# thu-ml/stochastic_gcn

Hardware: AMD Instinct MI355X
Metric: training edges/s (SpMM) (higher is better)
Workload: dtype f32

## Files before the change

### stochastic_gcn_amd/csrc/sgcn_gemm.hip

```cpp
#include "sgcn_dev.h"
#include "sgcn_bwd.h"

namespace sgcn {

typedef float f16acc __attribute__((ext_vector_type(16)));

constexpr int kTM = 32, kTN = 128, kTK = 32;

struct GemmArgs {
    const float* A; int64_t lda;
    const float* B; int64_t ldb;
    float* C; int64_t ldc;
    int32_t M, N, K;
    int32_t accumulate;
    int32_t kchunk;
    float* ws;
    const float* offset; const float* scale; float eps; int32_t relu;
    float* xhat; float* rstd;
    int32_t epi;
    const float* A2; int64_t lda2; int32_t a_split;
    DropArgs drop_a;
    DropArgs drop_c;
    int32_t vec_a, vec_b;
    const int32_t* a_gidx;
    const int32_t* a_gidx2;
};

__device__ __forceinline__ float wsum(float v) {
#pragma unroll
    for (int o = 32; o > 0; o >>= 1) v += __shfl_xor(v, o, 64);
    return v;
}

constexpr int kAsFloats = kTM * (kTK + 1), kBsFloats = kTK * (kTN + 4);
constexpr int kGroupFloats = kAsFloats + kBsFloats;

template <bool TA, bool TB, int KG>
__device__ __forceinline__ void gemm_body(const GemmArgs& g, const int bx, const int by, const int bz) {
    extern __shared__ float smem[];
    const int kg = threadIdx.x / kBlock;
    const int tid = threadIdx.x % kBlock, lane = tid & 63, wave = tid >> 6;
    float (*As)[kTK + 1] = reinterpret_cast<float (*)[kTK + 1]>(smem + kg * kGroupFloats);
    float (*Bs)[kTN + 4] = reinterpret_cast<float (*)[kTN + 4]>(smem + kg * kGroupFloats + kAsFloats);
    const int m0 = bx * kTM, n0 = by * kTN;
    const int kbeg = bz * g.kchunk;
    const int kend = min(g.K, kbeg + g.kchunk);
    f16acc acc = {};
    float ra[4], rb[16];
    float ep_scale[2] = {1.f, 1.f}, ep_offset[2] = {0.f, 0.f};
    if (g.epi == 2) {
#pragma unroll
        for (int e = 0; e < 2; e++) {
            const int c = (threadIdx.x & 63) + e * kWave;
            if (c < g.N) { ep_scale[e] = g.scale[c]; ep_offset[e] = g.offset[c]; }
        }
    }

    auto ld4 = [&](const float* rowp, bool vec, bool rowok, int first, int limit, float* out) {
        if (vec) {
            const bool ok = rowok && first + 3 < limit;
            const float4 v = *reinterpret_cast<const float4*>(rowp + (ok ? first : 0));
            out[0] = ok ? v.x : 0.f; out[1] = ok ? v.y : 0.f; out[2] = ok ? v.z : 0.f; out[3] = ok ? v.w : 0.f;
        } else {
#pragma unroll
            for (int e = 0; e < 4; e++) {
                const bool ok = rowok && first + e < limit;
                const float v = rowp[ok ? first + e : 0];
                out[e] = ok ? v : 0.f;
            }
        }
    };
    const float* arow = nullptr;
    if (!TA) {
        const int row = min(m0 + (tid >> 3), g.M - 1);
        if (g.A2 && row >= g.a_split) {
            const int r2 = row - g.a_split;
            arow = g.A2 + (int64_t)(g.a_gidx2 ? g.a_gidx2[r2] : r2) * g.lda2;
        } else {
            arow = g.A + (int64_t)(g.a_gidx ? g.a_gidx[row] : row) * g.lda;
        }
    }
    auto fetch = [&](int k0) {
        if (!TA) {
            const int i = tid >> 3, kq = (tid & 7) * 4, row = m0 + i;
            ld4(arow, g.vec_a, row < g.M, k0 + kq, kend, ra);
            if (g.drop_a.on) {
#pragma unroll
                for (int e = 0; e < 4; e++) ra[e] *= drop_factor(g.drop_a, row, k0 + kq + e);
            }
        } else {
            const int kk = tid >> 3, iq = (tid & 7) * 4, k = k0 + kk, kc = min(k, kend - 1);
            const int64_t ak = g.a_gidx ? g.a_gidx[kc] : kc;
            ld4(g.A + ak * g.lda, g.vec_a, k < kend, m0 + iq, g.M, ra);
            if (g.drop_a.on) {
#pragma unroll
                for (int e = 0; e < 4; e++) ra[e] *= drop_factor(g.drop_a, k, m0 + iq + e);
            }
        }
        if (!TB) {
#pragma unroll
            for (int r = 0; r < 4; r++) {
                const int kk = (tid >> 5) + 8 * r, jq = (tid & 31) * 4, k = k0 + kk;
                ld4(g.B + (int64_t)min(k, kend - 1) * g.ldb, g.vec_b, k < kend, n0 + jq, g.N, rb + r * 4);
            }
        } else {
#pragma unroll
            for (int r = 0; r < 4; r++) {
                const int j = (tid >> 3) + 32 * r, kq = (tid & 7) * 4, col = n0 + j;
                ld4(g.B + (int64_t)min(col, g.N - 1) * g.ldb, g.vec_b, col < g.N, k0 + kq, kend, rb + r * 4);
            }
        }
    };
    auto stage = [&]() {
        if (!TA) {
            const int i = tid >> 3, kq = (tid & 7) * 4;
#pragma unroll
            for (int e = 0; e < 4; e++) As[i][kq + e] = ra[e];
        } else {
            const int kk = tid >> 3, iq = (tid & 7) * 4;
#pragma unroll
            for (int e = 0; e < 4; e++) As[iq + e][kk] = ra[e];
        }
        if (!TB) {
#pragma unroll
            for (int r = 0; r < 4; r++) {
                const int kk = (tid >> 5) + 8 * r, jq = (tid & 31) * 4;
                *reinterpret_cast<float4*>(&Bs[kk][jq]) = make_float4(rb[r * 4], rb[r * 4 + 1], rb[r * 4 + 2], rb[r * 4 + 3]);
            }
        } else {
#pragma unroll
            for (int r = 0; r < 4; r++) {
                const int j = (tid >> 3) + 32 * r, kq = (tid & 7) * 4;
#pragma unroll
                for (int e = 0; e < 4; e++) Bs[kq + e][j] = rb[r * 4 + e];
            }
        }
    };

    const int iters = ((kend - kbeg + kTK - 1) / kTK + KG - 1) / KG;
    if (iters > 0) fetch(kbeg + kg * kTK);
    for (int it = 0; it < iters; it++) {
        const int k0 = kbeg + (it * KG + kg) * kTK;
        stage();
        __syncthreads();
        if (it + 1 < iters) fetch(k0 + KG * kTK);
        const int fi = lane & 31, fk = lane >> 5;
#pragma unroll
        for (int kk2 = 0; kk2 < kTK / 2; kk2++) {
            const float a = As[fi][kk2 * 2 + fk];
            const float b = Bs[kk2 * 2 + fk][wave * 32 + fi];
            acc = __builtin_amdgcn_mfma_f32_32x32x2f32(a, b, acc, 0, 0, 0);
        }
        __syncthreads();
    }

    const int cj = wave * 32 + (lane & 31);
    if (KG > 1) {
        if (kg > 0) {
#pragma unroll
            for (int r = 0; r < 16; r++) Bs[(r & 3) + 8 * (r >> 2) + 4 * (lane >> 5)][cj] = acc[r];
        }
        __syncthreads();
        if (kg == 0) {
            for (int o = 1; o < KG; o++) {
                float (*P)[kTN + 4] = reinterpret_cast<float (*)[kTN + 4]>(smem + o * kGroupFloats + kAsFloats);
#pragma unroll
                for (int r = 0; r < 16; r++) acc[r] += P[(r & 3) + 8 * (r >> 2) + 4 * (lane >> 5)][cj];
            }
        }
    }
    if (g.epi == 0) {
        if (kg != 0) return;
        float* base = g.ws ? g.ws + (int64_t)bz * g.M * g.N : g.C;
        const int64_t ld = g.ws ? g.N : g.ldc;
        const bool add = !g.ws && g.accumulate;
#pragma unroll
        for (int r = 0; r < 16; r++) {
            const int row = m0 + (r & 3) + 8 * (r >> 2) + 4 * (lane >> 5), col = n0 + cj;
            if (row < g.M && col < g.N) {
                float* p = base + (int64_t)row * ld + col;
                float v = acc[r];
                if (g.drop_c.on) v *= drop_factor(g.drop_c, row, col);
                *p = add ? *p + v : v;
            }
        }
        return;
    }
    float (*Cs)[kTN + 4] = reinterpret_cast<float (*)[kTN + 4]>(smem + kAsFloats);
    if (KG > 1) __syncthreads();
    if (kg == 0) {
#pragma unroll
        for (int r = 0; r < 16; r++) Cs[(r & 3) + 8 * (r >> 2) + 4 * (lane >> 5)][cj] = acc[r];
    }
    __syncthreads();
    for (int rr = kg * (kBlock / kWave) + wave; rr < kTM; rr += KG * (kBlock / kWave)) {
        const int row = m0 + rr;
        if (row >= g.M) break;
        float* yr = g.C + (int64_t)row * g.ldc;
        if (g.epi == 1) {
            for (int c = lane; c < g.N; c += kWave) { const float v = Cs[rr][c]; yr[c] = g.relu ? fmaxf(v, 0.f) : v; }
            continue;
        }
        float s = 0.f;
        for (int c = lane; c < g.N; c += kWave) s += Cs[rr][c];
        const float mean = wsum(s) / (float)g.N;
        float q = 0.f;
        for (int c = lane; c < g.N; c += kWave) { const float t = Cs[rr][c] - mean; q += t * t; }
        const float rs = rsqrtf(wsum(q) / (float)g.N + g.eps);
        if (lane == 0) g.rstd[row] = rs;
        float* hr = g.xhat + (int64_t)row * g.N;
#pragma unroll
        for (int e = 0; e < 2; e++) {
            const int c = lane + e * kWave;
            if (c < g.N) {
                const float h = (Cs[rr][c] - mean) * rs;
                hr[c] = h;
                const float v = h * ep_scale[e] + ep_offset[e];
                yr[c] = g.relu ? fmaxf(v, 0.f) : v;
            }
        }
    }
}

template <bool TA, bool TB, int KG>
__global__ __launch_bounds__(kBlock * KG) void gemm_kernel(GemmArgs g) {
    gemm_body<TA, TB, KG>(g, (int)blockIdx.x, (int)blockIdx.y, (int)blockIdx.z);
}

struct GemmGroup {
    GemmArgs g[kMaxGroup];
    int32_t first[kMaxGroup + 1];
    int32_t gx[kMaxGroup], gy[kMaxGroup];
    int32_t n;
};

template <bool TA, bool TB, int KG>
__global__ __launch_bounds__(kBlock * KG) void gemm_group_kernel(GemmGroup G) {
    const int b = (int)blockIdx.x;
    int j = 0;
#pragma unroll
    for (int q = 1; q < kMaxGroup; q++) j += (q < G.n && b >= G.first[q]) ? 1 : 0;
    const int l = b - G.first[j];
    const int gx = G.gx[j], gy = G.gy[j];
    gemm_body<TA, TB, KG>(G.g[j], l % gx, (l / gx) % gy, l / (gx * gy));
}

__global__ void splitk_reduce_kernel(const float* __restrict__ ws, int32_t S, int32_t M, int32_t N,
                                     float* __restrict__ C, int64_t ldc, int32_t accumulate) {
    const int64_t i = (int64_t)blockIdx.x * blockDim.x + threadIdx.x;
    const int64_t mn = (int64_t)M * N;
    if (i >= mn) return;
    float s = 0.f;
    for (int z = 0; z < S; z++) s += ws[(int64_t)z * mn + i];
    float* p = C + (i / N) * ldc + (i % N);
    *p = accumulate ? *p + s : s;
}

__global__ void dense_bwd_reduce_kernel(ReduceJob j, int32_t gemm_blocks, const float* __restrict__ ln_partial,
                                        int32_t nblk, int32_t d, float* __restrict__ doffset,
                                        float* __restrict__ dscale, int32_t ln_accumulate) {
    if ((int)blockIdx.x < gemm_blocks) {
        const int64_t i = (int64_t)blockIdx.x * blockDim.x + threadIdx.x;
        const int64_t mn = (int64_t)j.M * j.N;
        if (i >= mn) return;
        float s = 0.f;
        for (int z = 0; z < j.S; z++) s += j.ws[(int64_t)z * mn + i];
        float* p = j.C + (i / j.N) * j.ldc + (i % j.N);
        *p = j.accumulate ? *p + s : s;
    } else {
        ln_param_reduce_cols32(ln_partial, nblk, d, doffset, dscale, (int)blockIdx.x - gemm_blocks, ln_accumulate != 0);
    }
}

__global__ void dense_bwd_reduce_multi_kernel(ReduceMulti R) { reduce_multi_body(R, (int)blockIdx.x, nullptr); }

__global__ __launch_bounds__(kBlock) void splitk_ln_act_kernel(const float* __restrict__ ws, int32_t S,
                                                               GemmArgs g) {
    const int lane = threadIdx.x & 63;
    const int64_t row = (int64_t)blockIdx.x * (kBlock / kWave) + threadIdx.x / kWave;
    if (row >= g.M) return;
    const int64_t mn = (int64_t)g.M * g.N;
    float v[2];
    float sc[2] = {1.f, 1.f}, of[2] = {0.f, 0.f};
    if (g.epi == 2) {
#pragma unroll
        for (int e = 0; e < 2; e++) {
            const int c = lane + e * kWave;
            if (c < g.N) { sc[e] = g.scale[c]; of[e] = g.offset[c]; }
        }
    }
#pragma unroll
    for (int e = 0; e < 2; e++) {
        const int c = lane + e * kWave;
        float s = 0.f;
        if (c < g.N)
            for (int z = 0; z < S; z++) s += ws[(int64_t)z * mn + row * g.N + c];
        v[e] = s;
    }
    float* yr = g.C + row * g.ldc;
    if (g.epi == 2) {
        const float mean = wsum(v[0] + v[1]) / (float)g.N;
        float q = 0.f;
#pragma unroll
        for (int e = 0; e < 2; e++) if (lane + e * kWave < g.N) { const float t = v[e] - mean; q += t * t; }
        const float rs = rsqrtf(wsum(q) / (float)g.N + g.eps);
        if (lane == 0) g.rstd[row] = rs;
#pragma unroll
        for (int e = 0; e < 2; e++) {
            const int c = lane + e * kWave;
            if (c < g.N) {
                const float h = (v[e] - mean) * rs;
                g.xhat[row * g.N + c] = h;
                const float y = h * sc[e] + of[e];
                yr[c] = g.relu ? fmaxf(y, 0.f) : y;
            }
        }
    } else {
#pragma unroll
        for (int e = 0; e < 2; e++) {
            const int c = lane + e * kWave;
            if (c < g.N) yr[c] = (g.epi == 1 && g.relu) ? fmaxf(v[e], 0.f) : v[e];
        }
    }
}


struct RowDense {
    const float* W; int64_t ldw; int32_t N, kg;
    const float* offset; const float* scale; float eps; int32_t relu, epi;
    DropArgs drop;
    float* Y; int64_t ldy; float* xhat; float* rstd;
};

__global__ __launch_bounds__(kBlock) void splitk_ln_dense_kernel(const float* __restrict__ ws, int32_t S, GemmArgs g, RowDense d) {
    extern __shared__ __attribute__((aligned(1024))) float wl[];
    const int lane = threadIdx.x & 63;
    const int64_t row = (int64_t)blockIdx.x * (kBlock / kWave) + threadIdx.x / kWave;
    const bool live = row < g.M;
    const int K2 = g.N, total = K2 * d.N;
    {
        const int total4 = total / 4, wave = threadIdx.x >> 6;
        for (int base4 = wave * kWave; base4 < total4; base4 += (kBlock / kWave) * kWave) {
            const int i4 = min(base4 + lane, total4 - 1);
            __builtin_amdgcn_global_load_lds((const __attribute__((address_space(1))) void*)(d.W + (int64_t)i4 * 4),
                                             (__attribute__((address_space(3))) void*)(wl + (int64_t)base4 * 4), 16, 0, 0);
        }
    }
    float sc1[2] = {1.f, 1.f}, of1[2] = {0.f, 0.f}, sc2[2] = {1.f, 1.f}, of2[2] = {0.f, 0.f};
#pragma unroll
    for (int e = 0; e < 2; e++) {
        const int c = lane + e * kWave;
        if (g.epi == 2 && c < g.N) { sc1[e] = g.scale[c]; of1[e] = g.offset[c]; }
        if (d.epi == 2 && c < d.N) { sc2[e] = d.scale[c]; of2[e] = d.offset[c]; }
    }
    const int64_t mn = (int64_t)g.M * g.N;
    float v[2] = {0.f, 0.f};
    if (live) {
#pragma unroll
        for (int e = 0; e < 2; e++) {
            const int c = lane + e * kWave;
            float s = 0.f;
            if (c < g.N)
                for (int z = 0; z < S; z++) s += ws[(int64_t)z * mn + row * g.N + c];
            v[e] = s;
        }
    }
    asm volatile("s_waitcnt vmcnt(0)" ::: "memory");
    __syncthreads();
    if (!live) return;
    float x[2];
    float* yr = g.C + row * g.ldc;
    if (g.epi == 2) {
        const float mean = wsum(v[0] + v[1]) / (float)g.N;
        float q = 0.f;
#pragma unroll
        for (int e = 0; e < 2; e++) if (lane + e * kWave < g.N) { const float t = v[e] - mean; q += t * t; }
        const float rs = rsqrtf(wsum(q) / (float)g.N + g.eps);
        if (lane == 0) g.rstd[row] = rs;
#pragma unroll
        for (int e = 0; e < 2; e++) {
            const int c = lane + e * kWave;
            x[e] = 0.f;
            if (c < g.N) {
                const float h = (v[e] - mean) * rs;
                g.xhat[row * g.N + c] = h;
                const float y = h * sc1[e] + of1[e];
                x[e] = g.relu ? fmaxf(y, 0.f) : y;
                yr[c] = x[e];
            }
        }
    } else {
#pragma unroll
        for (int e = 0; e < 2; e++) {
            const int c = lane + e * kWave;
            x[e] = 0.f;
            if (c < g.N) { x[e] = (g.epi == 1 && g.relu) ? fmaxf(v[e], 0.f) : v[e]; yr[c] = x[e]; }
        }
    }
    if (d.drop.on) { x[0] *= drop_factor(d.drop, (int)row, lane); x[1] *= drop_factor(d.drop, (int)row, lane + kWave); }
    const int c0 = lane < d.N ? lane : 0, c1 = lane + kWave < d.N ? lane + kWave : 0;
    float a0[2] = {0.f, 0.f}, a1[2] = {0.f, 0.f};
    for (int s0 = 0; s0 * 32 < K2; s0++) {
        const int gi = d.kg > 1 ? (s0 & 1) : 0;
        const float xs = s0 < 2 ? x[0] : x[1];
        const int kb = s0 * 32, lb = kb & (kWave - 1);
        const float* wk = wl + kb * d.N;
        float p0 = a0[gi], p1 = a1[gi];
        if (kb + 32 <= K2) {
#pragma unroll
            for (int q = 0; q < 4; q++) {
                float w0[8], w1[8];
#pragma unroll
                for (int u = 0; u < 8; u++) { w0[u] = wk[(q * 8 + u) * d.N + c0]; w1[u] = wk[(q * 8 + u) * d.N + c1]; }
#pragma unroll
                for (int u = 0; u < 8; u++) {
                    const float xv = __int_as_float(__builtin_amdgcn_readlane(__float_as_int(xs), lb + q * 8 + u));
                    p0 = fmaf(xv, w0[u], p0); p1 = fmaf(xv, w1[u], p1);
                }
            }
        } else {
            for (int kk = 0; kb + kk < K2; kk++) {
                const float xv = __int_as_float(__builtin_amdgcn_readlane(__float_as_int(xs), lb + kk));
                p0 = fmaf(xv, wk[kk * d.N + c0], p0); p1 = fmaf(xv, wk[kk * d.N + c1], p1);
            }
        }
        a0[gi] = p0; a1[gi] = p1;
    }
    const float z[2] = {d.kg > 1 ? a0[0] + a0[1] : a0[0], d.kg > 1 ? a1[0] + a1[1] : a1[0]};
    float* y2 = d.Y + row * d.ldy;
    if (d.epi != 2) {
#pragma unroll
        for (int e = 0; e < 2; e++) {
            const int c = lane + e * kWave;
            if (c < d.N) y2[c] = (d.epi == 1 && d.relu) ? fmaxf(z[e], 0.f) : z[e];
        }
        return;
    }
    float s = 0.f;
#pragma unroll
    for (int e = 0; e < 2; e++) if (lane + e * kWave < d.N) s += z[e];
    const float mean = wsum(s) / (float)d.N;
    float q = 0.f;
#pragma unroll
    for (int e = 0; e < 2; e++) if (lane + e * kWave < d.N) { const float t = z[e] - mean; q += t * t; }
    const float rs = rsqrtf(wsum(q) / (float)d.N + d.eps);
    if (lane == 0) d.rstd[row] = rs;
#pragma unroll
    for (int e = 0; e < 2; e++) {
        const int c = lane + e * kWave;
        if (c < d.N) {
            const float h = (z[e] - mean) * rs;
            d.xhat[row * d.N + c] = h;
            const float y = h * sc2[e] + of2[e];
            y2[c] = d.relu ? fmaxf(y, 0.f) : y;
        }
    }
}

}

using namespace sgcn;

static int split_factor(int M, int N, int K) {
    const int tiles = ((M + kTM - 1) / kTM) * ((N + kTN - 1) / kTN);
    int s = 256 / std::max(tiles, 1);
    const int min_steps = tune_get("gemm_min_steps") > 0 ? tune_get("gemm_min_steps") : 3;
    s = std::min(s, K / (min_steps * kTK));
    return std::max(s, 1);
}

template <bool TA, bool TB, int KG>
static void launch_one(const GemmArgs& g, dim3 grid, hipStream_t st) {
    const size_t lds = (size_t)KG * kGroupFloats * sizeof(float);
    static bool raised = false;
    if (lds > 64 * 1024 && !raised) {
        (void)hipFuncSetAttribute(reinterpret_cast<const void*>(&gemm_kernel<TA, TB, KG>),
                                  hipFuncAttributeMaxDynamicSharedMemorySize, (int)lds);
        raised = true;
    }
    hipLaunchKernelGGL((gemm_kernel<TA, TB, KG>), grid, dim3(kBlock * KG), lds, st, g);
}

template <bool TA, bool TB>
static void launch_kg(const GemmArgs& g, dim3 grid, int kgroups, hipStream_t st) {
    if (kgroups >= 4) launch_one<TA, TB, 4>(g, grid, st);
    else if (kgroups == 2) launch_one<TA, TB, 2>(g, grid, st);
    else launch_one<TA, TB, 1>(g, grid, st);
}

struct GemmPlan { dim3 grid; int kgroups, S, epi; };

static GemmPlan prepare_gemm(GemmArgs& g, float* ws, int ta = 0, int tb = 0) {
    auto al = [](const void* p, int64_t ld) { return p && ((uintptr_t)p % 16 == 0) && (ld % 4 == 0); };
    g.vec_a = al(g.A, g.lda) && (!g.A2 || al(g.A2, g.lda2)) && (ta ? g.M : g.K) % 4 == 0;
    g.vec_b = al(g.B, g.ldb) && (tb ? g.K : g.N) % 4 == 0;
    int S = ws ? split_factor(g.M, g.N, g.K) : 1;
    g.kchunk = ((g.K + S - 1) / S + kTK - 1) / kTK * kTK;
    S = g.K > 0 ? (g.K + g.kchunk - 1) / g.kchunk : 1;
    if (g.K == 0) g.kchunk = kTK;
    g.ws = S > 1 ? ws : nullptr;
    GemmPlan p;
    p.epi = g.epi;
    p.S = S;
    if (S > 1) g.epi = 0;
    p.grid = dim3((unsigned)((g.M + kTM - 1) / kTM), (unsigned)((g.N + kTN - 1) / kTN), (unsigned)S);
    const int steps = (std::min(g.kchunk, g.K) + kTK - 1) / kTK;
    const int blocks = (int)(p.grid.x * p.grid.y * p.grid.z);
    p.kgroups = (blocks <= 128 && steps >= 8) ? 4 : ((blocks <= 256 && steps >= 4) ? 2 : 1);
    return p;
}

namespace sgcn {
void gemm_fwd_shape(int M, int N, int K, int* S, int* kgroups, int* kchunk) {
    GemmArgs g{};
    g.M = M; g.N = N; g.K = K;
    float dummy;
    const GemmPlan p = prepare_gemm(g, sgcn_gemm_ws_floats(M, N, K) > 0 ? &dummy : nullptr);
    *S = p.S; *kgroups = p.kgroups;
    if (kchunk) *kchunk = g.kchunk;
}
}

static void launch_prepared(const GemmArgs& g, const GemmPlan& p, int ta, int tb, hipStream_t st) {
    if (!ta && !tb) launch_kg<false, false>(g, p.grid, p.kgroups, st);
    else if (ta && !tb) launch_kg<true, false>(g, p.grid, p.kgroups, st);
    else if (!ta && tb) launch_kg<false, true>(g, p.grid, p.kgroups, st);
    else launch_kg<true, true>(g, p.grid, p.kgroups, st);
}

static int launch_gemm(GemmArgs g, int ta, int tb, float* ws, hipStream_t st, ReduceJob* defer = nullptr) {
    if (defer) defer->pending = 0;
    const GemmPlan p = prepare_gemm(g, ws, ta, tb);
    const int S = p.S, epi = p.epi;
    launch_prepared(g, p, ta, tb, st);
    if (S > 1 && epi != 0) {
        g.epi = epi;
        const unsigned rb = (unsigned)((g.M + (kBlock / kWave) - 1) / (kBlock / kWave));
        hipLaunchKernelGGL(splitk_ln_act_kernel, dim3(rb), dim3(kBlock), 0, st, g.ws, S, g);
    } else if (S > 1 && defer) {
        *defer = ReduceJob{g.ws, S, g.M, g.N, g.C, g.ldc, g.accumulate, 1};
    } else if (S > 1) {
        const int64_t mn = (int64_t)g.M * g.N;
        hipLaunchKernelGGL(splitk_reduce_kernel, dim3((unsigned)((mn + 255) / 256)), dim3(256), 0, st,
                           g.ws, S, g.M, g.N, g.C, g.ldc, g.accumulate);
    }
    SGCN_HIP_TRY(hipGetLastError());
    return SGCN_OK;
}

extern "C" int64_t sgcn_gemm_ws_floats(int32_t M, int32_t N, int32_t K) {
    if (M <= 0 || N <= 0 || K <= 0) return 0;
    const int S = split_factor(M, N, K);
    return S > 1 ? (int64_t)S * M * N : 0;
}

extern "C" int sgcn_gemm_f32(int32_t trans_a, int32_t trans_b, int32_t M, int32_t N, int32_t K,
                             const float* A, int64_t lda, const float* B, int64_t ldb, float* C,
                             int64_t ldc, int32_t accumulate, float* ws,
                             const sgcn_dropout_t* drop_a, const sgcn_dropout_t* drop_c, void* stream) {
    SGCN_REQUIRE(M >= 0 && N >= 0 && K >= 0, "gemm: negative size");
    if (M == 0 || N == 0) return SGCN_OK;
    SGCN_REQUIRE(C && (K == 0 || (A && B)), "gemm: null operand");
    GemmArgs g{};
    g.A = A; g.lda = lda; g.B = B; g.ldb = ldb; g.C = C; g.ldc = ldc;
    g.M = M; g.N = N; g.K = K; g.accumulate = accumulate; g.epi = 0;
    g.drop_a = drop_args(drop_a);
    g.drop_c = drop_args(drop_c);
    SGCN_REQUIRE(!g.drop_a.on || g.drop_a.width == (trans_a ? M : K), "gemm: drop_a width must be the stored A's row length");
    SGCN_REQUIRE(!g.drop_c.on || g.drop_c.width == N, "gemm: drop_c width must be N");
    if (g.drop_c.on) ws = nullptr;
    return launch_gemm(g, trans_a, trans_b, ws, (hipStream_t)stream);
}


namespace sgcn {
int dense_fwd_pair(int32_t M, int32_t N, int32_t K, const float* X, int64_t ldx, const float* X2, int64_t ldx2, int32_t split,
                   const float* W, int64_t ldw, const float* offset, const float* scale, float eps, int32_t relu, float* Y,
                   int64_t ldy, float* xhat, float* rstd, const sgcn_dropout_t* drop, float* ws, const int32_t* gidx,
                   const int32_t* gidx2, int32_t N2, const float* W2, int64_t ldw2, const float* offset2, const float* scale2,
                   float eps2, int32_t relu2, float* Y2, int64_t ldy2, float* xhat2, float* rstd2, const sgcn_dropout_t* drop2,
                   void* stream, int* fused) {
    *fused = 0;
    if (M <= 0 || N <= 0 || N > kTN || N2 <= 0 || N2 > kTN || !ws || !W2 || !Y2 || ldw2 != N2 || ldy != N) return SGCN_OK;
    const int norm = (offset && scale) ? 1 : 0, norm2 = (offset2 && scale2) ? 1 : 0;
    if ((norm && !(xhat && rstd)) || (norm2 && !(xhat2 && rstd2))) return SGCN_OK;
    GemmArgs g{};
    g.A = X; g.lda = ldx; g.B = W; g.ldb = ldw; g.C = Y; g.ldc = ldy;
    g.M = M; g.N = N; g.K = K; g.offset = offset; g.scale = scale; g.eps = eps; g.relu = relu;
    g.xhat = xhat; g.rstd = rstd; g.epi = norm ? 2 : (relu ? 1 : 0);
    g.A2 = X2; g.lda2 = ldx2; g.a_split = split;
    g.a_gidx = gidx; g.a_gidx2 = gidx2;
    g.drop_a = drop_args(drop);
    const GemmPlan p = prepare_gemm(g, ws);
    int S2 = 0, kg2 = 0;
    gemm_fwd_shape(M, N2, N, &S2, &kg2, nullptr);
    if (p.S <= 1 || S2 != 1 || kg2 > 2 || (size_t)N * N2 * sizeof(float) > 64 * 1024 || (N * N2) % 4 || !aligned16(W2)) return SGCN_OK;
    SGCN_REQUIRE(!g.drop_a.on || g.drop_a.width == K, "dense_fwd: dropout width must be K");
    RowDense d{};
    d.W = W2; d.ldw = ldw2; d.N = N2; d.kg = kg2; d.offset = offset2; d.scale = scale2; d.eps = eps2; d.relu = relu2;
    d.epi = norm2 ? 2 : (relu2 ? 1 : 0);
    d.drop = drop_args(drop2);
    SGCN_REQUIRE(!d.drop.on || d.drop.width == N, "dense_fwd: the second layer's dropout width must be its input width");
    d.Y = Y2; d.ldy = ldy2; d.xhat = xhat2; d.rstd = rstd2;
    hipStream_t st = (hipStream_t)stream;
    launch_prepared(g, p, 0, 0, st);
    g.epi = p.epi;
    const unsigned rb = (unsigned)((g.M + (kBlock / kWave) - 1) / (kBlock / kWave));
    hipLaunchKernelGGL(splitk_ln_dense_kernel, dim3(rb), dim3(kBlock), ((size_t)N * N2 + 255) / 256 * 256 * sizeof(float), st, g.ws, p.S, g, d);
    SGCN_HIP_TRY(hipGetLastError());
    *fused = 1;
    return SGCN_OK;
}
}

extern "C" int sgcn_dense_fwd_f32(int32_t M, int32_t N, int32_t K, const float* X, int64_t ldx,
                                  const float* X2, int64_t ldx2, int32_t split,
                                  const float* W, int64_t ldw, const float* offset,
                                  const float* scale, float eps, int32_t relu, float* Y, int64_t ldy,
                                  float* xhat, float* rstd, const sgcn_dropout_t* drop, float* ws,
                                  const int32_t* gidx, const int32_t* gidx2, void* stream) {
    SGCN_REQUIRE(M >= 0 && N >= 0 && K >= 0, "dense_fwd: negative size");
    if (M == 0 || N == 0) return SGCN_OK;
    SGCN_REQUIRE((X || (X2 && split == 0)) && W && Y, "dense_fwd: null operand");
    const int norm = (offset && scale) ? 1 : 0;
    SGCN_REQUIRE(!norm || (xhat && rstd), "dense_fwd: LayerNorm needs xhat / rstd");
    SGCN_REQUIRE(N <= kTN || (!norm && !relu), "dense_fwd: fused epilogue needs N <= 128");
    GemmArgs g{};
    g.A = X; g.lda = ldx; g.B = W; g.ldb = ldw; g.C = Y; g.ldc = ldy;
    g.M = M; g.N = N; g.K = K; g.offset = offset; g.scale = scale; g.eps = eps; g.relu = relu;
    g.xhat = xhat; g.rstd = rstd; g.epi = norm ? 2 : (relu ? 1 : 0);
    SGCN_REQUIRE(!X2 || (split >= 0 && split <= M), "dense_fwd: bad split");
    g.A2 = X2; g.lda2 = ldx2; g.a_split = split;
    g.a_gidx = gidx; g.a_gidx2 = gidx2;
    g.drop_a = drop_args(drop);
    SGCN_REQUIRE(!g.drop_a.on || g.drop_a.width == K, "dense_fwd: dropout width must be K");
    return launch_gemm(g, 0, 0, N <= kTN ? ws : nullptr, (hipStream_t)stream);
}


namespace sgcn {
namespace {
struct AuxCtx {
    hipStream_t st = nullptr;
    hipEvent_t fork = nullptr, join = nullptr;
    float* ring = nullptr;
    int64_t cap = 0, off = 0, want = 0;
    bool pending = false;
};
AuxCtx& aux_ctx() { static AuxCtx c; return c; }
int g_dw_recorded = 0;
int g_grad_store = 0;

int aux_init(AuxCtx& c) {
    if (c.st) return SGCN_OK;
    SGCN_HIP_TRY(hipStreamCreateWithFlags(&c.st, hipStreamNonBlocking));
    SGCN_HIP_TRY(hipEventCreateWithFlags(&c.fork, hipEventDisableTiming));
    SGCN_HIP_TRY(hipEventCreateWithFlags(&c.join, hipEventDisableTiming));
    return SGCN_OK;
}
}

int aux_fork(void* stream, void** aux_stream) {
    AuxCtx& c = aux_ctx();
    const int rc = aux_init(c);
    if (rc != SGCN_OK) return rc;
    SGCN_HIP_TRY(hipEventRecord(c.fork, (hipStream_t)stream));
    SGCN_HIP_TRY(hipStreamWaitEvent(c.st, c.fork, 0));
    c.pending = true;
    *aux_stream = (void*)c.st;
    return SGCN_OK;
}

bool reduce_parked();
int aux_join(void* stream) {
    AuxCtx& c = aux_ctx();
    if (c.pending) {
        SGCN_HIP_TRY(hipEventRecord(c.join, c.st));
        SGCN_HIP_TRY(hipStreamWaitEvent((hipStream_t)stream, c.join, 0));
        c.pending = false;
    }
    if (g_dw_recorded > 0 || reduce_parked()) return SGCN_OK;
    c.off = 0;
    if (c.want > c.cap) {
        SGCN_HIP_TRY(hipStreamSynchronize(c.st));
        if (c.ring) SGCN_HIP_TRY(hipFree(c.ring));
        c.ring = nullptr;
        c.cap = 0;
        const int64_t cap = c.want + c.want / 2;
        SGCN_HIP_TRY(hipMalloc((void**)&c.ring, (size_t)cap * sizeof(float)));
        c.cap = cap;
    }
    c.want = 0;
    return SGCN_OK;
}

struct BwdScratch { float* ws_ln; float* ws_dw; float* ws_gemm; hipStream_t st_dw; bool deferred; };

namespace {
struct DwJob { GemmArgs q; GemmPlan p; ReduceJob rj; const float* ws_ln; int32_t nblk, N; float* doffset; float* dscale; };
struct DwGroupState { DwJob jobs[kMaxGroup]; int n = 0; bool active = false; };
DwGroupState& dw_state() { static DwGroupState s; return s; }
}

void grad_store_mode(int on) { g_grad_store = on; }

int dw_group_begin() {
    DwGroupState& d = dw_state();
    d.n = 0;
    d.active = true;
    return SGCN_OK;
}

template <int KG>
static void launch_group(const GemmGroup& G, unsigned blocks, hipStream_t st) {
    const size_t lds = (size_t)KG * kGroupFloats * sizeof(float);
    static bool raised = false;
    if (lds > 64 * 1024 && !raised) {
        (void)hipFuncSetAttribute(reinterpret_cast<const void*>(&gemm_group_kernel<true, false, KG>),
                                  hipFuncAttributeMaxDynamicSharedMemorySize, (int)lds);
        raised = true;
    }
    hipLaunchKernelGGL((gemm_group_kernel<true, false, KG>), dim3(blocks), dim3(kBlock * KG), lds, st, G);
}

void dw_group_abort() {
    DwGroupState& d = dw_state();
    d.active = false;
    d.n = 0;
    g_dw_recorded = 0;
}

bool reduce_park(const ReduceMulti& R, int blocks);
int dw_group_flush(void* stream, bool park_reduce) {
    DwGroupState& d = dw_state();
    d.active = false;
    const int n = d.n;
    d.n = 0;
    g_dw_recorded = 0;
    if (n == 0) return SGCN_OK;
    hipStream_t st = (hipStream_t)stream;
    bool uniform = true;
    for (int k = 1; k < n; k++) uniform = uniform && d.jobs[k].p.kgroups == d.jobs[0].p.kgroups;
    if (uniform && n > 1) {
        GemmGroup G{};
        G.n = n;
        int first = 0;
        for (int k = 0; k < n; k++) {
            G.g[k] = d.jobs[k].q;
            G.first[k] = first;
            G.gx[k] = (int32_t)d.jobs[k].p.grid.x; G.gy[k] = (int32_t)d.jobs[k].p.grid.y;
            first += (int)(d.jobs[k].p.grid.x * d.jobs[k].p.grid.y * d.jobs[k].p.grid.z);
        }
        for (int k = n; k <= kMaxGroup; k++) G.first[k] = first;
        const int kg = d.jobs[0].p.kgroups;
        if (kg >= 4) launch_group<4>(G, (unsigned)first, st);
        else if (kg == 2) launch_group<2>(G, (unsigned)first, st);
        else launch_group<1>(G, (unsigned)first, st);
    } else {
        for (int k = 0; k < n; k++) launch_prepared(d.jobs[k].q, d.jobs[k].p, 1, 0, st);
    }
    ReduceMulti R{};
    R.n = n;
    R.ln_accumulate = g_grad_store ? 0 : 1;
    int b = 0;
    for (int k = 0; k < n; k++) {
        R.j[k] = d.jobs[k].rj;
        R.gfirst[k] = b;
        if (d.jobs[k].rj.pending) b += (int)(((int64_t)d.jobs[k].rj.M * d.jobs[k].rj.N + 255) / 256);
    }
    for (int k = n; k <= kMaxGroup; k++) R.gfirst[k] = b;
    for (int k = 0; k < n; k++) {
        R.ln_partial[k] = d.jobs[k].ws_ln; R.nblk[k] = d.jobs[k].nblk; R.d[k] = d.jobs[k].N;
        R.doffset[k] = d.jobs[k].doffset; R.dscale[k] = d.jobs[k].dscale;
        R.lfirst[k] = b;
        if (d.jobs[k].nblk > 0) b += (2 * d.jobs[k].N + kLnRedCols - 1) / kLnRedCols;
    }
    for (int k = n; k <= kMaxGroup; k++) R.lfirst[k] = b;
    if (b > 0 && !(park_reduce && reduce_park(R, b)))
        hipLaunchKernelGGL(dense_bwd_reduce_multi_kernel, dim3((unsigned)b), dim3(256), 0, st, R);
    SGCN_HIP_TRY(hipGetLastError());
    return SGCN_OK;
}

static int bwd_scratch(const DenseBwdArgs& a, hipStream_t st, bool overlap, BwdScratch& s) {
    const int64_t ln_floats = a.scale ? (sgcn_ln_act_bwd_ws_floats(a.n, a.N) + 3) / 4 * 4 : 0;
    s.ws_gemm = a.ws ? a.ws + ln_floats : nullptr;
    s.ws_ln = a.ws;
    s.ws_dw = s.ws_gemm;
    s.st_dw = st;
    s.deferred = false;
    if (dw_state().active && dw_state().n < kMaxGroup) {
        AuxCtx& c = aux_ctx();
        const int rc0 = aux_init(c);
        if (rc0 != SGCN_OK) return rc0;
        const int64_t need = ln_floats + (a.ws ? (sgcn_gemm_ws_floats(a.K, a.N, a.n) + 3) / 4 * 4 : 0);
        c.want += need;
        if (c.off + need <= c.cap) {
            if (a.ws) { s.ws_ln = c.ring + c.off; s.ws_dw = c.ring + c.off + ln_floats; }
            c.off += need;
            s.deferred = true;
        }
        return SGCN_OK;
    }
    if (overlap && a.dx) {
        AuxCtx& c = aux_ctx();
        const int rc0 = aux_init(c);
        if (rc0 != SGCN_OK) return rc0;
        const int64_t need = ln_floats + (a.ws ? (sgcn_gemm_ws_floats(a.K, a.N, a.n) + 3) / 4 * 4 : 0);
        c.want += need;
        if (c.off + need <= c.cap) {
            if (a.ws) { s.ws_ln = c.ring + c.off; s.ws_dw = c.ring + c.off + ln_floats; }
            c.off += need;
            s.st_dw = c.st;
        }
    }
    return SGCN_OK;
}

static int store_mode_zero(const DenseBwdArgs& a, void* stream) {
    if (!g_grad_store || a.N <= 0 || a.K <= 0) return SGCN_OK;
    hipStream_t st = (hipStream_t)stream;
    if (a.dW) SGCN_HIP_TRY(hipMemset2DAsync(a.dW, (size_t)a.lddw * sizeof(float), 0, (size_t)a.N * sizeof(float), (size_t)a.K, st));
    if (a.doffset) SGCN_HIP_TRY(hipMemsetAsync(a.doffset, 0, (size_t)a.N * sizeof(float), st));
    if (a.dscale) SGCN_HIP_TRY(hipMemsetAsync(a.dscale, 0, (size_t)a.N * sizeof(float), st));
    return SGCN_OK;
}

static int dense_bwd_run(const DenseBwdArgs& a, const BwdScratch& s, void* stream, const DenseBwdArgs* lower = nullptr,
                         const BwdScratch* slower = nullptr, bool* lower_done = nullptr, int32_t* lower_nblk = nullptr) {
    SGCN_REQUIRE(a.n >= 0 && a.N >= 0 && a.K >= 0, "dense_bwd: negative size");
    if (a.n == 0 || a.N == 0 || a.K == 0) return store_mode_zero(a, stream);
    SGCN_REQUIRE(a.dy && a.x && a.W && a.dW, "dense_bwd: null operand");
    hipStream_t st = (hipStream_t)stream;
    const float* g = a.dy;
    int64_t ldg = a.lddy;
    int32_t nblk = 0;
    bool dx_in_row_pass = false;
    int dx_kg = 1;
    if (lower_done && !lower && *lower_done) {
        nblk = lower_nblk ? *lower_nblk : 0;
        g = a.g_tmp; ldg = a.N;
    } else if (a.scale || a.relu) {
        SGCN_REQUIRE(a.g_tmp && a.y, "dense_bwd: LayerNorm / ReLU backward needs y and an n x N scratch");
        SGCN_REQUIRE(!a.scale || a.ws, "dense_bwd: LayerNorm backward needs the workspace");
        if (a.dx && (tune_get("step_fuse") & 8) && a.N <= 128 && a.N % 4 == 0 && a.K <= 256 && a.ldw == a.N && aligned16(a.W) &&
            (size_t)(8 * a.N + a.N * (a.K + 1)) * sizeof(float) <= 160 * 1024) {
            int S = 0, kgq = 0;
            const sgcn_dropout_t* dr = a.drop;
            if (dr && dr->keep >= 1.0f) dr = nullptr;
            if (dr) { S = 1; GemmArgs q{}; q.M = a.n; q.N = a.K; q.K = a.N; kgq = prepare_gemm(q, nullptr).kgroups; }
            else gemm_fwd_shape(a.n, a.K, a.N, &S, &kgq, nullptr);
            if (S == 1 && kgq <= 2) dx_in_row_pass = true, dx_kg = kgq;
        }
        const bool chain = dx_in_row_pass && lower && slower && lower_done && a.K <= 128 && lower->dy == a.dx && lower->lddy == a.lddx &&
                           lower->n == a.n && lower->N == a.K && (lower->scale || lower->relu) && lower->g_tmp && lower->y &&
                           (!lower->scale || (lower->xhat && lower->rstd && slower->ws_ln)) &&
                           (size_t)(8 * a.N + a.N * (a.K + 1) + 8 * a.K) * sizeof(float) <= 160 * 1024;
        const int rc = ln_act_bwd_launch(a.dy, a.lddy, a.y, a.ldy, a.xhat, a.rstd, a.scale, a.n, a.N, a.relu, a.g_tmp, a.N,
                                         a.doffset, a.dscale, s.ws_ln, false, &nblk, st,
                                         dx_in_row_pass ? a.W : nullptr, a.K, dx_kg, a.drop, a.dx, a.lddx,
                                         chain ? lower->y : nullptr, chain ? lower->ldy : 0, chain ? lower->xhat : nullptr,
                                         chain ? lower->rstd : nullptr, chain ? lower->scale : nullptr, chain ? lower->relu : 0,
                                         chain ? lower->g_tmp : nullptr, chain ? slower->ws_ln : nullptr);
        if (rc != SGCN_OK) return rc;
        if (chain) {
            *lower_done = true;
            if (lower_nblk) *lower_nblk = (lower->scale && a.scale) ? nblk : (lower->scale ? (a.n + 3) / 4 : 0);
        }
        g = a.g_tmp; ldg = a.N;
    }
    if (s.st_dw != st) {
        AuxCtx& c = aux_ctx();
        SGCN_HIP_TRY(hipEventRecord(c.fork, st));
        SGCN_HIP_TRY(hipStreamWaitEvent(c.st, c.fork, 0));
        c.pending = true;
    }
    GemmArgs q{};
    q.A = a.x; q.lda = a.ldx; q.B = g; q.ldb = ldg; q.C = a.dW; q.ldc = a.lddw;
    q.M = a.K; q.N = a.N; q.K = a.n; q.accumulate = g_grad_store ? 0 : 1; q.epi = 0;
    q.a_gidx = a.gidx;
    q.drop_a = drop_args(a.drop);
    SGCN_REQUIRE(!q.drop_a.on || q.drop_a.width == a.K, "dense_bwd: dropout width must be K");
    ReduceJob job{};
    int rc = SGCN_OK;
    if (s.deferred) {
        DwGroupState& dg = dw_state();
        DwJob& J = dg.jobs[dg.n++];
        g_dw_recorded = dg.n;
        J.q = q;
        J.p = prepare_gemm(J.q, s.ws_dw, 1, 0);
        J.rj = ReduceJob{J.q.ws, J.p.S, J.q.M, J.q.N, J.q.C, J.q.ldc, J.q.accumulate, J.p.S > 1 ? 1 : 0};
        J.ws_ln = s.ws_ln; J.nblk = nblk; J.N = a.N; J.doffset = a.doffset; J.dscale = a.dscale;
    } else {
        rc = launch_gemm(q, 1, 0, s.ws_dw, s.st_dw, &job);
        if (rc != SGCN_OK) return rc;
    }
    if (!s.deferred && (job.pending || nblk > 0)) {
        const int gb = job.pending ? (int)(((int64_t)job.M * job.N + 255) / 256) : 0;
        const int lb = nblk > 0 ? (2 * a.N + kLnRedCols - 1) / kLnRedCols : 0;
        hipLaunchKernelGGL(dense_bwd_reduce_kernel, dim3((unsigned)(gb + lb)), dim3(256), 0, s.st_dw, job, gb, s.ws_ln, nblk, a.N,
                           a.doffset, a.dscale, g_grad_store ? 0 : 1);
        SGCN_HIP_TRY(hipGetLastError());
    }
    if (!a.dx || dx_in_row_pass) return SGCN_OK;
    return sgcn_gemm_f32(0, 1, a.n, a.K, a.N, g, ldg, a.W, a.ldw, a.dx, a.lddx, 0, s.ws_gemm, nullptr, a.drop, stream);
}

static int dense_bwd_impl(int32_t n, int32_t N, int32_t K, const float* dy, int64_t lddy,
                          const float* y, int64_t ldy, const float* xhat, const float* rstd,
                          const float* scale, int32_t relu, const float* x, int64_t ldx,
                          const float* W, int64_t ldw, float* dW, int64_t lddw, float* doffset,
                          float* dscale, float* dx, int64_t lddx, const sgcn_dropout_t* drop,
                          float* g_tmp, float* ws, const int32_t* gidx, void* stream, bool overlap) {
    const DenseBwdArgs a{n, N, K, dy, lddy, y, ldy, xhat, rstd, scale, relu, x, ldx, W, ldw, dW, lddw, doffset, dscale,
                         dx, lddx, drop, g_tmp, ws, gidx};
    if (n == 0 || N == 0 || K == 0)
        return n >= 0 && N >= 0 && K >= 0 ? store_mode_zero(a, stream) : fail(SGCN_ERR_INVALID, "dense_bwd: negative size");
    BwdScratch s{};
    const int rc = bwd_scratch(a, (hipStream_t)stream, overlap, s);
    if (rc != SGCN_OK) return rc;
    return dense_bwd_run(a, s, stream);
}

int dense_bwd_chain(const DenseBwdArgs& up, const DenseBwdArgs& lo, void* stream) {
    const bool overlap = tune_get("step_overlap") != 0;
    if (up.n == 0 || up.N == 0 || up.K == 0 || lo.n == 0 || lo.N == 0 || lo.K == 0) {
        const int rz = store_mode_zero(up, stream);
        return rz != SGCN_OK ? rz : store_mode_zero(lo, stream);
    }
    BwdScratch su{}, sl{};
    int rc = bwd_scratch(up, (hipStream_t)stream, overlap, su);
    if (rc != SGCN_OK) return rc;
    rc = bwd_scratch(lo, (hipStream_t)stream, overlap, sl);
    if (rc != SGCN_OK) return rc;
    bool lower_done = false;
    int32_t lower_nblk = 0;
    const bool try_chain = (tune_get("step_fuse") & 64) && !lo.dx && su.deferred && sl.deferred;
    rc = dense_bwd_run(up, su, stream, try_chain ? &lo : nullptr, try_chain ? &sl : nullptr, &lower_done, &lower_nblk);
    if (rc != SGCN_OK) return rc;
    return dense_bwd_run(lo, sl, stream, nullptr, nullptr, &lower_done, &lower_nblk);
}

int dense_bwd_overlapped(int32_t n, int32_t N, int32_t K, const float* dy, int64_t lddy, const float* y, int64_t ldy,
                         const float* xhat, const float* rstd, const float* scale, int32_t relu, const float* x,
                         int64_t ldx, const float* W, int64_t ldw, float* dW, int64_t lddw, float* doffset,
                         float* dscale, float* dx, int64_t lddx, const sgcn_dropout_t* drop, float* g_tmp, float* ws,
                         const int32_t* gidx, void* stream) {
    return dense_bwd_impl(n, N, K, dy, lddy, y, ldy, xhat, rstd, scale, relu, x, ldx, W, ldw, dW, lddw, doffset, dscale,
                          dx, lddx, drop, g_tmp, ws, gidx, stream, tune_get("step_overlap") != 0);
}
}

extern "C" int sgcn_dense_bwd_f32(int32_t n, int32_t N, int32_t K, const float* dy, int64_t lddy,
                                  const float* y, int64_t ldy, const float* xhat, const float* rstd,
                                  const float* scale, int32_t relu, const float* x, int64_t ldx,
                                  const float* W, int64_t ldw, float* dW, int64_t lddw, float* doffset,
                                  float* dscale, float* dx, int64_t lddx, const sgcn_dropout_t* drop,
                                  float* g_tmp, float* ws, const int32_t* gidx, void* stream) {
    return sgcn::dense_bwd_impl(n, N, K, dy, lddy, y, ldy, xhat, rstd, scale, relu, x, ldx, W, ldw, dW, lddw, doffset,
                                dscale, dx, lddx, drop, g_tmp, ws, gidx, stream, false);
}
```

Before: 7.755 billion.

## Specialize GEMM on vector alignment and defer masking/dropout to stage

Result: no change. 7.755 billion (median of 4 runs) (-0.0%).

```diff
diff --git a/stochastic_gcn_amd/csrc/sgcn_gemm.hip b/stochastic_gcn_amd/csrc/sgcn_gemm.hip
--- a/stochastic_gcn_amd/csrc/sgcn_gemm.hip
+++ b/stochastic_gcn_amd/csrc/sgcn_gemm.hip
@@ -35,7 +35,7 @@
 constexpr int kAsFloats = kTM * (kTK + 1), kBsFloats = kTK * (kTN + 4);
 constexpr int kGroupFloats = kAsFloats + kBsFloats;
 
-template <bool TA, bool TB, int KG>
+template <bool TA, bool TB, int KG, bool VA, bool VB>
 __device__ __forceinline__ void gemm_body(const GemmArgs& g, const int bx, const int by, const int bz) {
     extern __shared__ float smem[];
     const int kg = threadIdx.x / kBlock;
@@ -56,20 +56,25 @@
         }
     }
 
-    auto ld4 = [&](const float* rowp, bool vec, bool rowok, int first, int limit, float* out) {
-        if (vec) {
+    auto ld4 = [&](auto vclass, const float* rowp, bool rowok, int first, int limit, float* out) {
+        if constexpr (decltype(vclass)::value) {
             const bool ok = rowok && first + 3 < limit;
             const float4 v = *reinterpret_cast<const float4*>(rowp + (ok ? first : 0));
-            out[0] = ok ? v.x : 0.f; out[1] = ok ? v.y : 0.f; out[2] = ok ? v.z : 0.f; out[3] = ok ? v.w : 0.f;
+            out[0] = v.x; out[1] = v.y; out[2] = v.z; out[3] = v.w;
         } else {
 #pragma unroll
-            for (int e = 0; e < 4; e++) {
-                const bool ok = rowok && first + e < limit;
-                const float v = rowp[ok ? first + e : 0];
-                out[e] = ok ? v : 0.f;
-            }
+            for (int e = 0; e < 4; e++) out[e] = rowp[(rowok && first + e < limit) ? first + e : 0];
         }
     };
+    auto sel4 = [&](auto vclass, bool rowok, int first, int limit, float* v) {
+#pragma unroll
+        for (int e = 0; e < 4; e++) {
+            const bool ok = rowok && first + (decltype(vclass)::value ? 3 : e) < limit;
+            v[e] = ok ? v[e] : 0.f;
+        }
+    };
+    constexpr std::integral_constant<bool, VA> va{};
+    constexpr std::integral_constant<bool, VB> vb{};
     const float* arow = nullptr;
     if (!TA) {
         const int row = min(m0 + (tid >> 3), g.M - 1);
@@ -80,44 +85,51 @@
             arow = g.A + (int64_t)(g.a_gidx ? g.a_gidx[row] : row) * g.lda;
         }
     }
+    int aidx = 0;
+    auto fetch_idx = [&](int k0) {
+        if (TA && g.a_gidx) aidx = g.a_gidx[min(k0 + (tid >> 3), kend - 1)];
+    };
     auto fetch = [&](int k0) {
         if (!TA) {
             const int i = tid >> 3, kq = (tid & 7) * 4, row = m0 + i;
-            ld4(arow, g.vec_a, row < g.M, k0 + kq, kend, ra);
-            if (g.drop_a.on) {
-#pragma unroll
-                for (int e = 0; e < 4; e++) ra[e] *= drop_factor(g.drop_a, row, k0 + kq + e);
-            }
+            ld4(va, arow, row < g.M, k0 + kq, kend, ra);
         } else {
             const int kk = tid >> 3, iq = (tid & 7) * 4, k = k0 + kk, kc = min(k, kend - 1);
-            const int64_t ak = g.a_gidx ? g.a_gidx[kc] : kc;
-            ld4(g.A + ak * g.lda, g.vec_a, k < kend, m0 + iq, g.M, ra);
-            if (g.drop_a.on) {
-#pragma unroll
-                for (int e = 0; e < 4; e++) ra[e] *= drop_factor(g.drop_a, k, m0 + iq + e);
-            }
+            const int64_t ak = g.a_gidx ? aidx : kc;
+            ld4(va, g.A + ak * g.lda, k < kend, m0 + iq, g.M, ra);
+            fetch_idx(k0 + KG * kTK);
         }
         if (!TB) {
 #pragma unroll
             for (int r = 0; r < 4; r++) {
                 const int kk = (tid >> 5) + 8 * r, jq = (tid & 31) * 4, k = k0 + kk;
-                ld4(g.B + (int64_t)min(k, kend - 1) * g.ldb, g.vec_b, k < kend, n0 + jq, g.N, rb + r * 4);
+                ld4(vb, g.B + (int64_t)min(k, kend - 1) * g.ldb, k < kend, n0 + jq, g.N, rb + r * 4);
             }
         } else {
 #pragma unroll
             for (int r = 0; r < 4; r++) {
                 const int j = (tid >> 3) + 32 * r, kq = (tid & 7) * 4, col = n0 + j;
-                ld4(g.B + (int64_t)min(col, g.N - 1) * g.ldb, g.vec_b, col < g.N, k0 + kq, kend, rb + r * 4);
+                ld4(vb, g.B + (int64_t)min(col, g.N - 1) * g.ldb, col < g.N, k0 + kq, kend, rb + r * 4);
             }
         }
     };
-    auto stage = [&]() {
+    auto stage = [&](int k0) {
         if (!TA) {
-            const int i = tid >> 3, kq = (tid & 7) * 4;
+            const int i = tid >> 3, kq = (tid & 7) * 4, row = m0 + i;
+            sel4(va, row < g.M, k0 + kq, kend, ra);
+            if (g.drop_a.on) {
+#pragma unroll
+                for (int e = 0; e < 4; e++) ra[e] *= drop_factor(g.drop_a, row, k0 + kq + e);
+            }
 #pragma unroll
             for (int e = 0; e < 4; e++) As[i][kq + e] = ra[e];
         } else {
-            const int kk = tid >> 3, iq = (tid & 7) * 4;
+            const int kk = tid >> 3, iq = (tid & 7) * 4, k = k0 + kk;
+            sel4(va, k < kend, m0 + iq, g.M, ra);
+            if (g.drop_a.on) {
+#pragma unroll
+                for (int e = 0; e < 4; e++) ra[e] *= drop_factor(g.drop_a, k, m0 + iq + e);
+            }
 #pragma unroll
             for (int e = 0; e < 4; e++) As[iq + e][kk] = ra[e];
         }
@@ -125,12 +137,14 @@
 #pragma unroll
             for (int r = 0; r < 4; r++) {
                 const int kk = (tid >> 5) + 8 * r, jq = (tid & 31) * 4;
+                sel4(vb, k0 + kk < kend, n0 + jq, g.N, rb + r * 4);
                 *reinterpret_cast<float4*>(&Bs[kk][jq]) = make_float4(rb[r * 4], rb[r * 4 + 1], rb[r * 4 + 2], rb[r * 4 + 3]);
             }
         } else {
 #pragma unroll
             for (int r = 0; r < 4; r++) {
                 const int j = (tid >> 3) + 32 * r, kq = (tid & 7) * 4;
+                sel4(vb, n0 + j < g.N, k0 + kq, kend, rb + r * 4);
 #pragma unroll
                 for (int e = 0; e < 4; e++) Bs[kq + e][j] = rb[r * 4 + e];
             }
@@ -138,10 +152,10 @@
     };
 
     const int iters = ((kend - kbeg + kTK - 1) / kTK + KG - 1) / KG;
-    if (iters > 0) fetch(kbeg + kg * kTK);
+    if (iters > 0) { fetch_idx(kbeg + kg * kTK); fetch(kbeg + kg * kTK); }
     for (int it = 0; it < iters; it++) {
         const int k0 = kbeg + (it * KG + kg) * kTK;
-        stage();
+        stage(k0);
         __syncthreads();
         if (it + 1 < iters) fetch(k0 + KG * kTK);
         const int fi = lane & 31, fk = lane >> 5;
@@ -222,9 +236,10 @@
     }
 }
 
-template <bool TA, bool TB, int KG>
-__global__ __launch_bounds__(kBlock * KG) void gemm_kernel(GemmArgs g) {
-    gemm_body<TA, TB, KG>(g, (int)blockIdx.x, (int)blockIdx.y, (int)blockIdx.z);
+template <bool TA, bool TB, int KG, bool VA, bool VB>
+__global__ __launch_bounds__(kBlock * KG) __attribute__((amdgpu_waves_per_eu((TA && TB) ? 5 : 6)))
+void gemm_kernel(GemmArgs g) {
+    gemm_body<TA, TB, KG, VA, VB>(g, (int)blockIdx.x, (int)blockIdx.y, (int)blockIdx.z);
 }
 
 struct GemmGroup {
@@ -234,7 +249,7 @@
     int32_t n;
 };
 
-template <bool TA, bool TB, int KG>
+template <bool TA, bool TB, int KG, bool VA, bool VB>
 __global__ __launch_bounds__(kBlock * KG) void gemm_group_kernel(GemmGroup G) {
     const int b = (int)blockIdx.x;
     int j = 0;
@@ -242,7 +257,7 @@
     for (int q = 1; q < kMaxGroup; q++) j += (q < G.n && b >= G.first[q]) ? 1 : 0;
     const int l = b - G.first[j];
     const int gx = G.gx[j], gy = G.gy[j];
-    gemm_body<TA, TB, KG>(G.g[j], l % gx, (l / gx) % gy, l / (gx * gy));
+    gemm_body<TA, TB, KG, VA, VB>(G.g[j], l % gx, (l / gx) % gy, l / (gx * gy));
 }
 
 __global__ void splitk_reduce_kernel(const float* __restrict__ ws, int32_t S, int32_t M, int32_t N,
@@ -469,16 +484,24 @@
     return std::max(s, 1);
 }
 
-template <bool TA, bool TB, int KG>
-static void launch_one(const GemmArgs& g, dim3 grid, hipStream_t st) {
+template <bool TA, bool TB, int KG, bool VA, bool VB>
+static void launch_class(const GemmArgs& g, dim3 grid, hipStream_t st) {
     const size_t lds = (size_t)KG * kGroupFloats * sizeof(float);
     static bool raised = false;
     if (lds > 64 * 1024 && !raised) {
-        (void)hipFuncSetAttribute(reinterpret_cast<const void*>(&gemm_kernel<TA, TB, KG>),
+        (void)hipFuncSetAttribute(reinterpret_cast<const void*>(&gemm_kernel<TA, TB, KG, VA, VB>),
                                   hipFuncAttributeMaxDynamicSharedMemorySize, (int)lds);
         raised = true;
     }
-    hipLaunchKernelGGL((gemm_kernel<TA, TB, KG>), grid, dim3(kBlock * KG), lds, st, g);
+    hipLaunchKernelGGL((gemm_kernel<TA, TB, KG, VA, VB>), grid, dim3(kBlock * KG), lds, st, g);
+}
+
+template <bool TA, bool TB, int KG>
+static void launch_one(const GemmArgs& g, dim3 grid, hipStream_t st) {
+    if (g.vec_a && g.vec_b) launch_class<TA, TB, KG, true, true>(g, grid, st);
+    else if (g.vec_a) launch_class<TA, TB, KG, true, false>(g, grid, st);
+    else if (g.vec_b) launch_class<TA, TB, KG, false, true>(g, grid, st);
+    else launch_class<TA, TB, KG, false, false>(g, grid, st);
 }
 
 template <bool TA, bool TB>
@@ -711,16 +734,26 @@
     return SGCN_OK;
 }
 
-template <int KG>
-static void launch_group(const GemmGroup& G, unsigned blocks, hipStream_t st) {
+template <int KG, bool VA, bool VB>
+static void launch_group_class(const GemmGroup& G, unsigned blocks, hipStream_t st) {
     const size_t lds = (size_t)KG * kGroupFloats * sizeof(float);
     static bool raised = false;
     if (lds > 64 * 1024 && !raised) {
-        (void)hipFuncSetAttribute(reinterpret_cast<const void*>(&gemm_group_kernel<true, false, KG>),
+        (void)hipFuncSetAttribute(reinterpret_cast<const void*>(&gemm_group_kernel<true, false, KG, VA, VB>),
                                   hipFuncAttributeMaxDynamicSharedMemorySize, (int)lds);
         raised = true;
     }
-    hipLaunchKernelGGL((gemm_group_kernel<true, false, KG>), dim3(blocks), dim3(kBlock * KG), lds, st, G);
+    hipLaunchKernelGGL((gemm_group_kernel<true, false, KG, VA, VB>), dim3(blocks), dim3(kBlock * KG), lds, st, G);
+}
+
+template <int KG>
+static void launch_group(const GemmGroup& G, unsigned blocks, hipStream_t st) {
+    bool va = true, vb = true;
+    for (int k = 0; k < G.n; k++) { va = va && G.g[k].vec_a; vb = vb && G.g[k].vec_b; }
+    if (va && vb) launch_group_class<KG, true, true>(G, blocks, st);
+    else if (va) launch_group_class<KG, true, false>(G, blocks, st);
+    else if (vb) launch_group_class<KG, false, true>(G, blocks, st);
+    else launch_group_class<KG, false, false>(G, blocks, st);
 }
 
 void dw_group_abort() {
```
